# Arlo0o/StereoScene

Hardware: AMD Instinct MI355X
Metric: voxels/sec fwd+bwd, 256x256x32 grid D=192 (higher is better)
Workload: dtype f32; 1 GPU; kitti_d192: stereo pair features 2x[B,640,48,160] -> 256x256x32 occupancy, D=192, fwd+bwd incl. 4 losses; batch_per_gpu=1, global_batch=1, parallelism=dp1, train_mode=True

## Files before the change

include/ssbev.h:

```cpp
#ifndef SSBEV_H
#define SSBEV_H

#include <stddef.h>
#include <stdint.h>

#ifdef __cplusplus
extern "C" {
#endif

#define SSBEV_OK 0
#define SSBEV_EINVAL (-1)
#define SSBEV_EWORKSPACE (-2)
#define SSBEV_ELAUNCH (-3)

typedef void* ssbev_stream_t;

int ssbev_version(void);
const char* ssbev_build_arch(void);
void ssbev_env_refresh(void);

typedef struct {
  int B;
  int P;
  int C;
// ... 337 lines not shown
size_t ssbev_wino_dgemm_packed_elems(int Cout, int Cin);
int ssbev_wino_dgemm_pack(const float* w, float* Wp, int Cout, int Cin, int mode, ssbev_stream_t stream);
int ssbev_wino_dgemm(const float* P, const float* Wp, float* Mo, const ssbev_wino_dims* d, int N, ssbev_stream_t stream);
int ssbev_wino_bgemm(const float* A, const float* Wp, float* Cm, int64_t T, int K, int N, ssbev_stream_t stream);

typedef struct {
  int M, N, K, batch;
  int64_t lda, ldb, ldc, sa, sb, sc;
  int relu;
  int d2s_D, d2s_H, d2s_W, d2s_kd, d2s_kh, d2s_kw, d2s_Co;
  const int64_t* d2s_rowoff;
  const float* ep_mul;
  const float* ep_rowsub;
} ssbev_gemm_dims;
int ssbev_gemm_d2s_rowoff(int64_t* rowoff, int M, int D, int H, int W, int kd, int kh, int kw, int Co, ssbev_stream_t stream);
size_t ssbev_gemm_nn_workspace(const ssbev_gemm_dims* d);
size_t ssbev_gemm_nt_workspace(const ssbev_gemm_dims* d);
int ssbev_gemm_nn(const float* A, const float* B, const float* bias, float* C, const ssbev_gemm_dims* d, void* workspace,
                  size_t ws_bytes, ssbev_stream_t stream);
int ssbev_gemm_nt(const float* A, const float* W, const float* bias, float* C, const ssbev_gemm_dims* d, void* workspace,
                  size_t ws_bytes, ssbev_stream_t stream);
size_t ssbev_gemm_tn_workspace(const ssbev_gemm_dims* d);
int ssbev_gemm_tn(const float* A, const float* B, float* C, const ssbev_gemm_dims* d, void* workspace, size_t ws_bytes,
                  ssbev_stream_t stream);
typedef struct {
  int kernel;
  int bm, bn, bk;
  int nchunk;
  int per_chunk;
  int64_t grid;
  size_t workspace;
} ssbev_gemm_plan;
int ssbev_gemm_plan_query(const ssbev_gemm_dims* d, int form, ssbev_gemm_plan* out);

int ssbev_wino43_df_supported(const ssbev_wino_dims* d, int N);
int ssbev_wino43_df_instance(const ssbev_wino_dims* d, int N);
size_t ssbev_wino43_df_packed_elems(int Cout, int Cin);
int ssbev_wino43_df_pack(const float* w, float* Wp, int Cout, int Cin, int mode, ssbev_stream_t stream);
int ssbev_wino43_df_gemm(const float* P, const float* Wp, float* Mo, const ssbev_wino_dims* d, int N, ssbev_stream_t stream);
size_t ssbev_wino43_df_wgrad_workspace(const ssbev_wino_dims* d, int N);
int ssbev_wino43_df_wgrad(const float* P, const float* Z, float* gw, const ssbev_wino_dims* d, int N, void* workspace,
                          size_t ws_bytes, ssbev_stream_t stream);
typedef struct {
  int mt, nw;
  int ncolgrp, nrowgrp;
  int nst;
  int64_t grid;
  size_t lds_bytes;
  int w_kw, w_nt, w_br;
  int w_nkb, w_nnb;
  int w_nchunk;
  int w_stages_per_chunk;
  int w_total_stages;
  int64_t w_grid;
  size_t w_lds_bytes;
  size_t w_workspace;
} ssbev_wino43_df_plan;
int ssbev_wino43_df_plan_query(const ssbev_wino_dims* d, int N, ssbev_wino43_df_plan* out);

#ifdef __cplusplus
}
#endif
#endif
```

stereoscene_amd/capi.py:

```python
import ctypes as C
import os

import torch

_HERE = os.path.dirname(os.path.abspath(__file__))
LIB_PATH = os.path.join(_HERE, "_lib", "libssbev_hip.so")

OK, EINVAL, EWORKSPACE, ELAUNCH = 0, -1, -2, -3
_ERR = {EINVAL: "SSBEV_EINVAL (bad dims / null pointer / unsupported configuration)",
        EWORKSPACE: "SSBEV_EWORKSPACE (workspace too small)",
        ELAUNCH: "SSBEV_ELAUNCH (HIP launch failure)"}


class SsbevError(RuntimeError):
    pass


class PoolDims(C.Structure):
    _fields_ = [("B", C.c_int), ("P", C.c_int), ("C", C.c_int), ("nx", C.c_int), ("ny", C.c_int), ("nz", C.c_int),
                ("origin", C.c_float * 3), ("dx", C.c_float * 3)]


class LiftDims(C.Structure):
    _fields_ = [("N", C.c_int), ("D", C.c_int), ("HW", C.c_int)]
# ... 178 lines not shown
    "ssbev_depth_bce_fwd": (C.c_int, [_P, _P, _P] + [C.c_int] * 5 + [C.c_float] * 3 + [_P, C.c_size_t, _P]),
    "ssbev_depth_bce_bwd": (C.c_int, [_P, _P, _P, _P] + [C.c_int] * 5 + [C.c_float] * 3 + [_P, _P]),
    "ssbev_depth_kld_workspace": (C.c_size_t, [C.c_int, C.c_int, C.c_int]),
    "ssbev_depth_kld_fwd": (C.c_int, [_P, _P, _P] + [C.c_int] * 5 + [C.c_double] * 3 + [C.c_float] * 3 + [_P, C.c_size_t, _P]),
    "ssbev_depth_kld_bwd": (C.c_int, [_P, _P, _P, _P] + [C.c_int] * 5 + [C.c_double] * 3 + [C.c_float] * 3 + [_P, C.c_size_t, _P]),
    "ssbev_lidar_depth_workspace": (C.c_size_t, [C.c_int, C.c_int]),
    "ssbev_lidar_depth_map": (C.c_int, [_P, C.c_int, _P, _P, _P, _P, _P, _P, C.c_int, C.c_int, _P, C.c_size_t, _P]),
    "ssbev_dwconv2d_fwd": (C.c_int, [_P, _P, _P, C.POINTER(DwDims), _P]),
    "ssbev_dwconv2d_bwd_data": (C.c_int, [_P, _P, _P, C.POINTER(DwDims), _P]),
    "ssbev_dwconv2d_bwd_weight_workspace": (C.c_size_t, [C.POINTER(DwDims)]),
    "ssbev_dwconv2d_bwd_weight": (C.c_int, [_P, _P, _P, C.POINTER(DwDims), _P, C.c_size_t, _P]),
    "ssbev_swish_fwd": (C.c_int, [_P, _P, C.c_int64, _P]),
    "ssbev_swish_bwd": (C.c_int, [_P, _P, _P, C.c_int64, _P]),
    "ssbev_chan_sum_workspace": (C.c_size_t, [C.c_int, C.c_int64, C.c_int]),
    "ssbev_chan_sum": (C.c_int, [_P, _P, _P, C.c_int, C.c_int64, C.c_int, C.c_float, _P, C.c_size_t, _P]),
    "ssbev_chan_scale": (C.c_int, [_P, _P, _P, C.c_int, C.c_int64, C.c_int, C.c_float, _P]),
    "ssbev_wino_input_transform": (C.c_int, [_P, _P, C.POINTER(WinoDims), _P]),
    "ssbev_wino_output_transform": (C.c_int, [_P, _P, C.POINTER(WinoDims), _P]),
    "ssbev_wino_output_adjoint": (C.c_int, [_P, _P, C.POINTER(WinoDims), _P]),
    "ssbev_wino_weight_transform": (C.c_int, [_P, _P, C.c_int, C.c_int, C.c_int, C.c_int, _P]),
    "ssbev_wino_weight_grad": (C.c_int, [_P, _P, C.c_int, C.c_int, C.c_int, _P]),
    "ssbev_wino_dgemm_packed_elems": (C.c_size_t, [C.c_int, C.c_int]),
    "ssbev_wino_dgemm_pack": (C.c_int, [_P, _P, C.c_int, C.c_int, C.c_int, _P]),
    "ssbev_wino_dgemm": (C.c_int, [_P, _P, _P, C.POINTER(WinoDims), C.c_int, _P]),
    "ssbev_wino_bgemm": (C.c_int, [_P, _P, _P, C.c_int64, C.c_int, C.c_int, _P]),
    "ssbev_gemm_d2s_rowoff": (C.c_int, [_P, C.c_int, C.c_int, C.c_int, C.c_int, C.c_int, C.c_int, C.c_int, C.c_int, _P]),
    "ssbev_gemm_nn_workspace": (C.c_size_t, [C.POINTER(GemmDims)]),
    "ssbev_gemm_nt_workspace": (C.c_size_t, [C.POINTER(GemmDims)]),
    "ssbev_gemm_nn": (C.c_int, [_P, _P, _P, _P, C.POINTER(GemmDims), _P, C.c_size_t, _P]),
    "ssbev_gemm_nt": (C.c_int, [_P, _P, _P, _P, C.POINTER(GemmDims), _P, C.c_size_t, _P]),
    "ssbev_gemm_tn_workspace": (C.c_size_t, [C.POINTER(GemmDims)]),
    "ssbev_gemm_tn": (C.c_int, [_P, _P, _P, C.POINTER(GemmDims), _P, C.c_size_t, _P]),
    "ssbev_gemm_plan_query": (C.c_int, [C.POINTER(GemmDims), C.c_int, C.POINTER(GemmPlan)]),
    "ssbev_wino43_df_supported": (C.c_int, [C.POINTER(WinoDims), C.c_int]),
    "ssbev_wino43_df_instance": (C.c_int, [C.POINTER(WinoDims), C.c_int]),
    "ssbev_wino43_df_packed_elems": (C.c_size_t, [C.c_int, C.c_int]),
    "ssbev_wino43_df_pack": (C.c_int, [_P, _P, C.c_int, C.c_int, C.c_int, _P]),
    "ssbev_wino43_df_gemm": (C.c_int, [_P, _P, _P, C.POINTER(WinoDims), C.c_int, _P]),
    "ssbev_wino43_df_wgrad_workspace": (C.c_size_t, [C.POINTER(WinoDims), C.c_int]),
    "ssbev_wino43_df_wgrad": (C.c_int, [_P, _P, _P, C.POINTER(WinoDims), C.c_int, _P, C.c_size_t, _P]),
    "ssbev_wino43_df_plan_query": (C.c_int, [C.POINTER(WinoDims), C.c_int, C.POINTER(Wino43DfPlan)]),
    "ssbev_wino2d_axis_tiles": (C.c_int, [C.c_int, C.c_int, C.POINTER(C.c_uint16), C.c_int]),
    "ssbev_wino2d_input_transform": (C.c_int, [_P, _P, C.POINTER(WinoDims), _P]),
    "ssbev_wino2d_output_transform": (C.c_int, [_P, _P, C.POINTER(WinoDims), _P]),
    "ssbev_wino2d_output_adjoint": (C.c_int, [_P, _P, C.POINTER(WinoDims), _P]),
    "ssbev_wino43_input_transform": (C.c_int, [_P, _P, C.POINTER(WinoDims), _P]),
    "ssbev_wino43_input_transform_bf16": (C.c_int, [_P, _P, C.POINTER(WinoDims), _P]),
    "ssbev_wino43_output_transform": (C.c_int, [_P, _P, C.POINTER(WinoDims), _P]),
    "ssbev_wino43_output_transform_bf16": (C.c_int, [_P, _P, C.POINTER(WinoDims), _P]),
    "ssbev_wino43_output_adjoint": (C.c_int, [_P, _P, C.POINTER(WinoDims), _P]),
    "ssbev_wino43_output_adjoint_bf16": (C.c_int, [_P, _P, C.POINTER(WinoDims), _P]),
    "ssbev_wino43_2d_input_transform": (C.c_int, [_P, _P, C.POINTER(WinoDims), _P]),
    "ssbev_wino43_2d_input_transform_bf16": (C.c_int, [_P, _P, C.POINTER(WinoDims), _P]),
    "ssbev_wino43_2d_output_transform": (C.c_int, [_P, _P, C.POINTER(WinoDims), _P]),
    "ssbev_wino43_2d_output_transform_acc": (C.c_int, [_P, _P, C.POINTER(WinoDims), _P]),
    "ssbev_wino2d_output_transform_acc": (C.c_int, [_P, _P, C.POINTER(WinoDims), _P]),
    "ssbev_wino43_2d_output_transform_bf16": (C.c_int, [_P, _P, C.POINTER(WinoDims), _P]),
    "ssbev_wino43_2d_output_adjoint": (C.c_int, [_P, _P, C.POINTER(WinoDims), _P]),
    "ssbev_wino43_2d_output_adjoint_bf16": (C.c_int, [_P, _P, C.POINTER(WinoDims), _P]),
    "ssbev_wino444_input_transform": (C.c_int, [_P, _P, C.POINTER(WinoDims), _P]),
    "ssbev_wino444_output_transform": (C.c_int, [_P, _P, C.POINTER(WinoDims), _P]),
    "ssbev_wino444_output_adjoint": (C.c_int, [_P, _P, C.POINTER(WinoDims), _P]),
    "ssbev_wino43_weight_transform": (C.c_int, [_P, _P, C.c_int, C.c_int, C.c_int, C.c_int, _P]),
    "ssbev_wino43_weight_grad": (C.c_int, [_P, _P, C.c_int, C.c_int, C.c_int, _P]),
    "ssbev_wino_input_transform_bf16": (C.c_int, [_P, _P, C.POINTER(WinoDims), _P]),
    "ssbev_wino_output_transform_bf16": (C.c_int, [_P, _P, C.POINTER(WinoDims), _P]),
# ... 86 lines not shown
```

stereoscene_amd/csrc/capi.hip:

```cpp
#include "common.h"

#include <cstdlib>
#include <mutex>
#include <string>
#include <unordered_map>

namespace {
struct EnvTable {
  std::mutex mu;
  std::unordered_map<std::string, std::pair<bool, std::string>> seen;
};
EnvTable& env_table() {
  static EnvTable* t = new EnvTable();
  return *t;
}
}

const char* ssbev_env(const char* name) {
  EnvTable& t = env_table();
  std::lock_guard<std::mutex> lock(t.mu);
  auto it = t.seen.find(name);
  if (it == t.seen.end()) {
    const char* v = std::getenv(name);
    it = t.seen.emplace(name, std::make_pair(v != nullptr, std::string(v ? v : ""))).first;
  }
  return it->second.first ? it->second.second.c_str() : nullptr;
}

extern "C" {
int ssbev_version(void) { return 112;  }
const char* ssbev_build_arch(void) { return "gfx950"; }

void ssbev_env_refresh(void) {
  EnvTable& t = env_table();
  std::lock_guard<std::mutex> lock(t.mu);
  t.seen.clear();
}
}
```

stereoscene_amd/csrc/gemm.hip:

```cpp
#include "common.h"

#include <algorithm>
#include <cstdlib>
#include <string>

namespace {

typedef float gf32x16 __attribute__((ext_vector_type(16)));
typedef float gv4f __attribute__((ext_vector_type(4)));
__device__ const float kGemmZeros[4] = {0.f, 0.f, 0.f, 0.f};

struct GemmGeom {
  int M, N, K, batch;
  long lda, ldb, ldc;
  long sa, sb, sc;
  int mblocks, nblocks;
  int nchunk, rows_per_chunk;
  int relu;
  int d2s_D, d2s_H, d2s_W, d2s_kd, d2s_kh, d2s_kw, d2s_Co;
  const long* rowoff;
  const float* ep_mul;
  const float* ep_rowsub;
};

// ... 364 lines not shown
      for (int kt = 0; kt < KT; ++kt)
#pragma unroll
        for (int r = 0; r < 16; ++r) {
          const int k = ko + kt * 32 + (r & 3) + 8 * (r >> 2) + 4 * lk;
          if (k < g.K && n < g.N) dst[(size_t)k * g.N + n] = acc[kt][nt][r];
        }
    }
    return;
  }
  __shared__ float fold[QUAD ? 1 : 4][KT * NT * 1024];
#pragma unroll
  for (int kt = 0; kt < KT; ++kt)
#pragma unroll
    for (int nt = 0; nt < NT; ++nt)
#pragma unroll
      for (int r = 0; r < 16; ++r) fold[wave][((kt * NT + nt) * 16 + r) * 64 + lane] = acc[kt][nt][r];
  __syncthreads();
  if (wave != 0) return;
#pragma unroll
  for (int nt = 0; nt < NT; ++nt) {
    const int n = nt * 32 + li;
#pragma unroll
    for (int kt = 0; kt < KT; ++kt)
#pragma unroll
      for (int r = 0; r < 16; ++r) {
        const int k = kt * 32 + (r & 3) + 8 * (r >> 2) + 4 * lk;
        const int o = ((kt * NT + nt) * 16 + r) * 64 + lane;
        const float v = ((fold[0][o] + fold[1][o]) + fold[2][o]) + fold[3][o];
        if (k < g.K && n < g.N) dst[(size_t)k * g.N + n] = v;
      }
  }
}

__global__ void __launch_bounds__(1024)
gemm_sum_wide_kernel(const float* __restrict__ part, float* __restrict__ out, size_t n, int nchunk) {
  __shared__ float red[16][64];
  const int e = threadIdx.x & 63, grp = threadIdx.x >> 6;
  const size_t i = (size_t)blockIdx.x * 64 + e;
  const int per = (nchunk + 15) / 16, c0 = grp * per, c1 = min(nchunk, c0 + per);
  float a = 0.0f;
  if (i < n)
    for (int c = c0; c < c1; ++c) a += part[(size_t)c * n + i];
  red[grp][e] = a;
  __syncthreads();
  if (grp == 0 && i < n) {
    float v = red[0][e];
#pragma unroll
    for (int q = 1; q < 16; ++q) v += red[q][e];
    out[i] = v;
  }
}

__global__ void __launch_bounds__(256)
gemm_sum_kernel(const float* __restrict__ part, float* __restrict__ out, size_t n, int nchunk, const float* __restrict__ bias,
                int N, int relu, long MN = 0, long ldc = 0, long sc = 0) {
  const size_t i = (size_t)blockIdx.x * 256 + threadIdx.x;
  if (i >= n) return;
  float a = part[i];
  for (int c = 1; c < nchunk; ++c) a += part[(size_t)c * n + i];
  if (bias) a += bias[i % N];
  if (relu) a = fmaxf(a, 0.0f);
  if (MN > 0) {
    const size_t b = i / MN, r = i - b * MN;
    out[b * sc + (r / N) * ldc + r % N] = a;
  } else {
    out[i] = a;
// ... 157 lines not shown

LaunchPlan plan_tn(const ssbev_gemm_dims* d) {
  LaunchPlan pl;
  if (tn_skinny(d)) {
    const int wgs = tn_skinny_wgs(d);
    const bool quad = tn_quad(d);
    const long runs = quad ? wgs : (long)wgs * 4;
    const int kt = quad ? 2 : (d->K + 31) / 32, nt = quad ? 2 : (d->N + 31) / 32;
    pl.mblocks = pl.nblocks = 1;
    pl.p.kernel = quad ? kTnSkinnyQuad : (kt == 1 ? (nt == 1 ? kTnSkinny11 : kTnSkinny12) : (nt == 1 ? kTnSkinny21 : kTnSkinny22));
    pl.p.bm = (quad ? 64 : 32) * kt; pl.p.bn = (quad ? 64 : 32) * nt; pl.p.bk = 16;
    pl.p.nchunk = wgs;
    pl.p.per_chunk = (int)(((long)d->M + runs - 1) / runs + 1) / 2 * 2;
    pl.p.grid = (int64_t)wgs * d->batch;
    pl.p.workspace = (size_t)wgs * d->batch * d->K * d->N * sizeof(float);
    return pl;
  }
  const int wn = pick_wn(d->N, d->d2s_kd > 0 ? d->d2s_Co : 0);
  const bool wide = tn_wide(d);
  const int BN = wide ? 160 : 64 * wn;
  pl.mblocks = (d->K + 127) / 128;
  pl.nblocks = (d->N + BN - 1) / BN;
  const int tiles = pl.mblocks * pl.nblocks;
  const int nchunk = d->ep_mul ? 1 : (wide ? tn_chunks_model(d, tiles) : tn_chunks(d, tiles));
  pl.p.kernel = wide ? kTnWide : (wn == 2 ? kTnPlain : kTnNarrow);
  pl.p.bm = 128; pl.p.bn = BN; pl.p.bk = 32;
  pl.p.nchunk = nchunk;
  pl.p.per_chunk = ((d->M + nchunk - 1) / nchunk + 31) / 32 * 32;
  pl.p.grid = (int64_t)d->batch * nchunk * tiles;
  pl.p.workspace = nchunk > 1 ? (size_t)nchunk * d->batch * d->K * d->N * sizeof(float) : 0;
  return pl;
}

bool nn_dims_ok(const ssbev_gemm_dims* d) {
  if (!gemm_ok(d) || d->lda < d->K || d->ldb < d->N) return false;
  return d->d2s_kd > 0 ? (d->batch == 1 && d->N == d->d2s_kd * d->d2s_kh * d->d2s_kw * d->d2s_Co) : d->ldc >= d->N;
}
bool nt_dims_ok(const ssbev_gemm_dims* d) {
  if (!gemm_ok(d) || d->ldb < d->K || d->ldc < d->N) return false;
  return d->d2s_kd > 0 ? (d->batch == 1 && d->K == d->d2s_kd * d->d2s_kh * d->d2s_kw * d->d2s_Co) : d->lda >= d->K;
}
bool tn_dims_ok(const ssbev_gemm_dims* d) {
  if (!gemm_ok(d) || d->lda < d->K) return false;
  if (d->d2s_kd > 0 ? (d->batch != 1 || d->N != d->d2s_kd * d->d2s_kh * d->d2s_kw * d->d2s_Co) : d->ldb < d->N) return false;
  if ((d->ep_mul != nullptr) != (d->ep_rowsub != nullptr)) return false;
  return !(d->ep_mul && (tn_skinny(d) || d->d2s_kd > 0));
}

template <bool BT>
int launch_nn(const float* A, const float* B, const float* bias, float* Cm, const ssbev_gemm_dims* d, void* ws, size_t ws_bytes,
              hipStream_t st) {
  GemmGeom g;
  fill_geom(g, d);
  const LaunchPlan pl = plan_nn<BT>(d);
  const int cfg = pl.p.kernel;
  const NnCfg& c = kNnCfgs[cfg];
  g.mblocks = pl.mblocks;
  g.nblocks = pl.nblocks;
  g.nchunk = pl.p.nchunk;
  g.rows_per_chunk = pl.p.per_chunk;
  float* dst = Cm;
  const float* kbias = bias;
  if (g.nchunk > 1) {
    if (!ws || ws_bytes < pl.p.workspace) return SSBEV_EWORKSPACE;
    dst = static_cast<float*>(ws);
    g.ldc = d->N; g.sc = (long)d->M * d->N; g.relu = 0;
// ... 83 lines not shown
      default: hipLaunchKernelGGL((gemm_tn_skinny_kernel<2, 2, false>), grid, block, 0, st, A, B, part, g, rows_per_run); break;
    }
    const size_t n = (size_t)d->batch * d->K * d->N;
    hipLaunchKernelGGL(gemm_sum_wide_kernel, dim3(cdiv(n, 64)), dim3(1024), 0, st, part, Cm, n, wgs);
    return ssbev_launch_status();
  }
  g.mblocks = pl.mblocks;
  g.nblocks = pl.nblocks;
  g.nchunk = pl.p.nchunk;
  g.rows_per_chunk = pl.p.per_chunk;
  float* dst = g.nchunk > 1 ? static_cast<float*>(ws) : Cm;
  const long nwg = (long)pl.p.grid;
  const size_t lds = (size_t)2 * (32 * 128 + 32 * pl.p.bn) * sizeof(float);
  if (pl.p.kernel == kTnWide) {
    auto kern = gemm_tn_kernel<5, 1, 1>;
    if (hipFuncSetAttribute(reinterpret_cast<const void*>(kern), hipFuncAttributeMaxDynamicSharedMemorySize, (int)lds) != hipSuccess)
      return SSBEV_ELAUNCH;
    hipLaunchKernelGGL(kern, dim3((unsigned)nwg), dim3(256), lds, st, A, B, dst, g);
  } else if (pl.p.kernel == kTnPlain) {
    auto kern = gemm_tn_kernel<2>;
    if (hipFuncSetAttribute(reinterpret_cast<const void*>(kern), hipFuncAttributeMaxDynamicSharedMemorySize, (int)lds) != hipSuccess)
      return SSBEV_ELAUNCH;
    hipLaunchKernelGGL(kern, dim3((unsigned)nwg), dim3(256), lds, st, A, B, dst, g);
  } else {
    hipLaunchKernelGGL(gemm_tn_kernel<1>, dim3((unsigned)nwg), dim3(256), lds, st, A, B, dst, g);
  }
  if (g.nchunk > 1) {
    const size_t n = (size_t)g.batch * d->K * d->N;
    hipLaunchKernelGGL(gemm_sum_kernel, dim3(cdiv(n, 256)), dim3(256), 0, st, dst, Cm, n, g.nchunk, (const float*)nullptr, 1, 0);
  }
  return ssbev_launch_status();
}

int ssbev_gemm_plan_query(const ssbev_gemm_dims* d, int form, ssbev_gemm_plan* out) {
  if (!out) return SSBEV_EINVAL;
  switch (form) {
    case 0: if (!nn_dims_ok(d)) return SSBEV_EINVAL; *out = plan_nn<false>(d).p; return SSBEV_OK;
    case 1: if (!nt_dims_ok(d)) return SSBEV_EINVAL; *out = plan_nn<true>(d).p; return SSBEV_OK;
    case 2: if (!tn_dims_ok(d)) return SSBEV_EINVAL; *out = plan_tn(d).p; return SSBEV_OK;
    default: return SSBEV_EINVAL;
  }
}

}
```

stereoscene_amd/functional.py:

```python
import ctypes as C
import math

import os

import numpy as np
import torch

from . import capi, streams



class KernelTimer:

    def __init__(self, families=None):
        self.records = []
        self.counts = {}
        self.families = families

    def span(self, family, flops, nbytes=0.0, tag=None, executed=None):
        c = self.counts.setdefault(family, dict(launches=0, flops=0.0, bytes=0.0, executed=0.0))
        c["launches"] += 1
        c["flops"] += flops
        c["bytes"] += nbytes
        c["executed"] += flops if executed is None else executed
# ... 508 lines not shown

    @staticmethod
    def backward(ctx, gy):
        lib = capi.load()
        xcl, weight = ctx.saved_tensors[:2]
        stride, padding, dilation, transposed, output_padding, kpad, has_bias = ctx.cfg
        args = (stride, padding, dilation, transposed, output_padding)
        if ctx.relu:
            ycl = ctx.saved_tensors[2]
            gy = from_cl(torch.ops.aten.threshold_backward(to_cl(gy).contiguous(), ycl, 0.0))
        gcl0 = to_cl(gy)
        Cout_g = gcl0.shape[-1]
        cpad = (-Cout_g) % 4
        tpad = (-xcl.shape[-1]) % 4 if ctx.thin_in else 0
        want_gx, want_gw = ctx.needs_input_grad[0], ctx.needs_input_grad[1]
        thin_d = thin_w = False
        d0 = None
        if not transposed and not kpad and (cpad or tpad):
            d0 = _conv_dims(tuple(xcl.shape), tuple(weight.shape), *args)
            thin_d = bool(cpad) and lib.ssbev_conv_kernel_class(C.byref(d0), 1) == 4
            thin_w = lib.ssbev_conv_kernel_class(C.byref(d0), 2) == 6
        w5 = weight.detach()
        if kpad:
            w5 = torch.nn.functional.pad(w5, (0, 0, 0, 0, 0, 0) + ((0, 0, 0, kpad) if transposed else (0, kpad)))
        gcl = gcl0
        if cpad and ((want_gx and not thin_d) or (want_gw and not thin_w)):
            gcl = torch.nn.functional.pad(gcl0, (0, cpad))
            w5 = torch.nn.functional.pad(w5, (0, 0, 0, 0, 0, 0) + ((0, cpad) if transposed else (0, 0, 0, cpad)))
        elif cpad:
            w5 = None
        d = _conv_dims(tuple(xcl.shape), tuple(w5.shape), *args) if w5 is not None else d0
        gx = gw = gb = None

        def weight_gradient():
            pointwise = (not transposed and tuple(weight.shape[2:]) == (1, 1, 1) and stride == (1, 1, 1) and padding == (0, 0, 0)
                         and not kpad and not cpad and not tpad and weight.shape[0] <= 128 and weight.shape[1] <= 128
                         and gcl0.numel() // Cout_g >= 32768)
            if pointwise and OWN_GEMM and PRECISION == "fp32":
                with _span("conv_wgrad", conv_flops(d), conv_bytes(d), _conv_tag(d, "wgrad")):
                    gw = gemm_tn(gcl0.reshape(-1, Cout_g), xcl.reshape(-1, xcl.shape[-1])).view_as(weight)
            else:
                if thin_w:
                    xw, gw_src, dw, wshape = xcl, gcl0, d0, tuple(weight.shape)
                else:
                    xw, gw_src, dw, wshape = xcl, gcl, d, tuple(w5.shape)
                    if tpad:
                        xw = torch.nn.functional.pad(xcl, (0, tpad))
                        wshape = (wshape[0], wshape[1] + tpad) + wshape[2:]
                        dw = _conv_dims(tuple(xw.shape), wshape, *args)
                gwp = torch.empty(wshape, dtype=torch.float32, device=gy.device)
                ws = _ws(lib.ssbev_conv_bwd_weight_workspace(C.byref(dw)), gy.device)
                with _span("conv_wgrad", conv_flops(dw), conv_bytes(dw), _conv_tag(dw, "wgrad")):
                    capi.check(lib.ssbev_conv_bwd_weight(capi.ptr(xw), capi.ptr(gw_src), capi.ptr(gwp), C.byref(dw),
                                                         capi.ptr(ws), ws.numel(), capi.stream()),
                               "ssbev_conv_bwd_weight")
                gw = gwp if tuple(wshape) == tuple(weight.shape) else gwp[: weight.shape[0], : weight.shape[1]].contiguous()
            return gw

        gw_side = want_gw and streams.wgrad_on_side(weight)
        want_gb = has_bias and ctx.needs_input_grad[2]
        gb_side = gw_side and want_gb and ctx.bias_leaf
        if gw_side:
            with streams.on_side(gy.device, xcl, gcl0, gcl) as side:
                gw = weight_gradient()
                if gb_side:
                    gb = gcl0.reshape(-1, Cout_g).sum(0)
                side.publish(gw, gb)
        if want_gx:
            dd, gdl, wd = (d0, gcl0, weight.detach()) if thin_d else (d, gcl, w5)
            slot = ctx.slot if (not kpad and not thin_d and lib.ssbev_conv_kernel_class(C.byref(dd), 1) not in (4, 5)) else None
            into = _slot_target(slot, xcl)
            if into is not None:
                dd.accumulate = 1
            gxcl = into if into is not None else torch.empty_like(xcl)
            fam = _conv_family(lib, dd, 1)
            with _span(fam, conv_flops(dd), conv_bytes(dd), _conv_tag(dd, "dgrad"), conv_flops(dd) / _EXEC_DIV[fam]):
                if lib.ssbev_conv_kernel_class(C.byref(dd), 1) == 5:
                    _thin_out_run(lib, gdl, wd, None, gxcl, dd, 1)
                else:
                    wpt = _packed(wd, dd, 1)
                    capi.check(lib.ssbev_conv_bwd_data(capi.ptr(gdl), capi.ptr(wpt), capi.ptr(gxcl), C.byref(dd),
                                                       capi.stream()), "ssbev_conv_bwd_data")
            dd.accumulate = 0
            if slot is not None:
                slot.buf = gxcl
            if kpad:
                gxcl = gxcl[..., : xcl.shape[-1] - kpad]
            gx = from_cl(gxcl)
        if want_gw and not gw_side:
            gw = weight_gradient()
        if want_gb and not gb_side:
            gb = gcl0.reshape(-1, Cout_g).sum(0)
        return gx, gw, gb, None, None, None, None, None, None, None


class _ConvNd16(torch.autograd.Function):

    @staticmethod
    def forward(ctx, x, weight, bias, stride, padding, dilation, transposed, output_padding, slot=None, relu=False, out_fp32=False):
        lib = capi.load()
        ctx.slot = slot
        if ctx.needs_input_grad[1]:
            streams.note_use(weight)
        xcl = to_cl(x if x.dtype == torch.bfloat16 else x.to(torch.bfloat16))
        d = _conv_dims(tuple(xcl.shape), tuple(weight.shape), stride, padding, dilation, transposed, output_padding, relu=int(relu))
        d.precision = 3 if out_fp32 else 2
        y = torch.empty(d.B, d.Do, d.Ho, d.Wo, d.Cout, dtype=torch.float32 if out_fp32 else torch.bfloat16, device=x.device)
        b = bias.detach().float().contiguous() if bias is not None else None
        fam = {17: "conv_tap16", 19: "conv_wide16"}.get(lib.ssbev_conv_kernel_class(C.byref(d), 0), "conv_gather16") if KERNEL_TIMER is not None else "conv_gather16"
        with _span(fam, conv_flops(d), conv_bytes(d) / 2.0, _conv_tag(d, "fwd")):
            wp = _packed(weight.detach(), d, 0)
            capi.check(lib.ssbev_conv_fwd_bf16(capi.ptr(xcl), capi.ptr(wp), capi.ptr(b), capi.ptr(y), C.byref(d), capi.stream()),
                       "ssbev_conv_fwd_bf16")
        ctx.relu = bool(relu)
        ctx.save_for_backward(xcl, weight, *((y,) if relu else ()))
        ctx.cfg = (stride, padding, dilation, transposed, output_padding, bias is not None)
        ctx.bias_leaf = bias is not None and bias.is_leaf and bias.grad is None
        return from_cl(y)

    @staticmethod
    def backward(ctx, gy):
        lib = capi.load()
        xcl, weight = ctx.saved_tensors[:2]
        stride, padding, dilation, transposed, output_padding, has_bias = ctx.cfg
# ... 199 lines not shown
    lib = capi.load()
    ws = _ws(lib.ssbev_gemm_nt_workspace(C.byref(g)), a.device)
    with _span("gemm_own", fl, 4.0 * (a.numel() + w.numel() + out.numel()), tag or f"nt {batch}x{M}x{K}x{N}"):
        capi.check(lib.ssbev_gemm_nt(_rawptr(a), _rawptr(w), _rawptr(bias.contiguous() if bias is not None else None),
                                     capi.ptr(out), C.byref(g), capi.ptr(ws), ws.numel(), capi.stream()), "ssbev_gemm_nt")
    return out


def gemm_tn(a, b, tag=None, ep_mul=None, ep_rowsub=None):
    if not _gemm_supported(a, b) or a.shape[-1] % 4 or b.shape[-1] % 4:
        c = torch.matmul(a.transpose(-1, -2), b)
        return c if ep_mul is None else ep_mul * (c - ep_rowsub.unsqueeze(-1))
    a, lda, sa = _rows(a)
    b, ldb, sb = _rows(b)
    batch = a.shape[0] if a.dim() == 3 else 1
    R, K, N = a.shape[-2], a.shape[-1], b.shape[-1]
    out = torch.empty(*a.shape[:-2], K, N, dtype=torch.float32, device=a.device)
    g = _gdims(R, N, K, batch, lda, ldb, N, sa, sb, K * N)
    if ep_mul is not None:
        ep_mul, ep_rowsub = ep_mul.contiguous(), ep_rowsub.contiguous().float()
        if tuple(ep_mul.shape) != tuple(out.shape) or ep_rowsub.numel() != batch * K:
            raise capi.SsbevError("gemm_tn: epilogue operand shapes")
        g.ep_mul, g.ep_rowsub = ep_mul.data_ptr(), ep_rowsub.data_ptr()
    lib = capi.load()
    ws = _ws(lib.ssbev_gemm_tn_workspace(C.byref(g)), a.device)
    fl = 2.0 * batch * R * N * K
    with _span("gemm_own", fl, 4.0 * (a.numel() + b.numel() + out.numel() * (2 if ep_mul is not None else 1)),
               tag or f"tn {batch}x{R}x{K}x{N}"):
        capi.check(lib.ssbev_gemm_tn(_rawptr(a), _rawptr(b), capi.ptr(out), C.byref(g), capi.ptr(ws), ws.numel(), capi.stream()),
                   "ssbev_gemm_tn")
    return out


class _LinearCL(torch.autograd.Function):

    @staticmethod
    def forward(ctx, x2, w2, bias):
        ctx.save_for_backward(x2, w2)
        ctx.has_bias = bias is not None
        return gemm_nt(x2, w2, bias, tag=f"linear fwd {w2.shape[1]}->{w2.shape[0]} rows={x2.shape[0]}")

    @staticmethod
    def backward(ctx, gy):
        x2, w2 = ctx.saved_tensors
        gy = gy.contiguous()
        gx = gw = gb = None
        if ctx.needs_input_grad[0]:
            gx = gemm_nn(gy, w2, tag=f"linear dgrad {w2.shape[1]}->{w2.shape[0]} rows={x2.shape[0]}")
        if ctx.needs_input_grad[1]:
            gw = gemm_tn(gy, x2, tag=f"linear wgrad {w2.shape[1]}->{w2.shape[0]} rows={x2.shape[0]}")
        if ctx.has_bias and ctx.needs_input_grad[2]:
            gb = gy.sum(0)
        return gx, gw, gb


_D2S_TABLES = {}


def _d2s_table(B, D, H, W, k, Co, device):
    key = (B, D, H, W, k, Co, str(device))
    t = _D2S_TABLES.get(key)
    if t is None:
        t = torch.empty(B * D * H * W, dtype=torch.int64, device=device)
        capi.check(capi.load().ssbev_gemm_d2s_rowoff(capi.ptr(t), B * D * H * W, D, H, W, k[0], k[1], k[2], Co, capi.stream()),
                   "ssbev_gemm_d2s_rowoff")
        _D2S_TABLES[key] = t
    return t


class _DeconvKS(torch.autograd.Function):

    @staticmethod
    def forward(ctx, xcl, weight, bias, k):
        B, D, H, W, Ci = xcl.shape
        Co = weight.shape[1]
        kd, kh, kw = k
        taps = kd * kh * kw
        wk = weight.detach().permute(0, 2, 3, 4, 1).reshape(Ci, taps * Co).contiguous()
        table = _d2s_table(B, D, H, W, k, Co, xcl.device)
        y = torch.empty(B, D * kd, H * kh, W * kw, Co, dtype=torch.float32, device=xcl.device)
        x2 = xcl.reshape(-1, Ci)
        R = x2.shape[0]
        g = _gdims(R, taps * Co, Ci, 1, Ci, taps * Co, 0, 0, 0, 0, 0, ((D, H, W, kd, kh, kw, Co), table))
        fl = 2.0 * R * Ci * taps * Co
# ... 1669 lines not shown
```

Baseline: 31.26 million voxels/s.

## Add fused pointwise weight-gradient kernel with bias-gradient column sums

Measured after the change: 31.28 million voxels/s, median of 6. No clear change (+0.1%).

```diff
diff --git a/include/ssbev.h b/include/ssbev.h
--- a/include/ssbev.h
+++ b/include/ssbev.h
@@ -393,6 +393,10 @@
   size_t workspace;
 } ssbev_gemm_plan;
 int ssbev_gemm_plan_query(const ssbev_gemm_dims* d, int form, ssbev_gemm_plan* out);
+size_t ssbev_wgrad_pointwise_workspace(const ssbev_gemm_dims* d);
+int ssbev_wgrad_pointwise_plan(const ssbev_gemm_dims* d, ssbev_gemm_plan* out);
+int ssbev_wgrad_pointwise(const float* A, const float* B, float* gw, float* gb, int gy_operand, const ssbev_gemm_dims* d,
+                          void* workspace, size_t ws_bytes, ssbev_stream_t stream);
 
 int ssbev_wino43_df_supported(const ssbev_wino_dims* d, int N);
 int ssbev_wino43_df_instance(const ssbev_wino_dims* d, int N);
diff --git a/stereoscene_amd/capi.py b/stereoscene_amd/capi.py
--- a/stereoscene_amd/capi.py
+++ b/stereoscene_amd/capi.py
@@ -234,6 +234,9 @@
     "ssbev_gemm_tn_workspace": (C.c_size_t, [C.POINTER(GemmDims)]),
     "ssbev_gemm_tn": (C.c_int, [_P, _P, _P, C.POINTER(GemmDims), _P, C.c_size_t, _P]),
     "ssbev_gemm_plan_query": (C.c_int, [C.POINTER(GemmDims), C.c_int, C.POINTER(GemmPlan)]),
+    "ssbev_wgrad_pointwise_workspace": (C.c_size_t, [C.POINTER(GemmDims)]),
+    "ssbev_wgrad_pointwise_plan": (C.c_int, [C.POINTER(GemmDims), C.POINTER(GemmPlan)]),
+    "ssbev_wgrad_pointwise": (C.c_int, [_P, _P, _P, _P, C.c_int, C.POINTER(GemmDims), _P, C.c_size_t, _P]),
     "ssbev_wino43_df_supported": (C.c_int, [C.POINTER(WinoDims), C.c_int]),
     "ssbev_wino43_df_instance": (C.c_int, [C.POINTER(WinoDims), C.c_int]),
     "ssbev_wino43_df_packed_elems": (C.c_size_t, [C.c_int, C.c_int]),
diff --git a/stereoscene_amd/csrc/capi.hip b/stereoscene_amd/csrc/capi.hip
--- a/stereoscene_amd/csrc/capi.hip
+++ b/stereoscene_amd/csrc/capi.hip
@@ -28,7 +28,7 @@
 }
 
 extern "C" {
-int ssbev_version(void) { return 112;  }
+int ssbev_version(void) { return 113;  }
 const char* ssbev_build_arch(void) { return "gfx950"; }
 
 void ssbev_env_refresh(void) {
diff --git a/stereoscene_amd/csrc/gemm.hip b/stereoscene_amd/csrc/gemm.hip
--- a/stereoscene_amd/csrc/gemm.hip
+++ b/stereoscene_amd/csrc/gemm.hip
@@ -420,6 +420,231 @@
   }
 }
 
+template <int KT, int NT, int WK, int WN>
+struct WgradPw {
+  static constexpr bool SHARED = WK * WN == 4;
+  static constexpr int KC = 32 * KT * WK, NC = 32 * NT * WN;
+  static constexpr int RS = SHARED ? ((KC == 32 || NC == 32) ? 32 : 16) : (KT * NT == 1 ? 16 : 8);
+  static constexpr int RW = SHARED ? RS / 4 : RS;
+  static constexpr int AF = RS * KC, BF = RS * NC, SF = AF + BF;
+  static constexpr int AP = RW * KC / 256, BP = RW * NC / 256, IPS = AP + BP;
+  static constexpr int NBUF = 3;
+  static constexpr int TILE = KT * NT * 1024;
+  static constexpr int STAGE_FLOATS = (SHARED ? 1 : 4) * NBUF * SF;
+  static constexpr int FOLD_FLOATS = SHARED ? 0 : 3 * TILE + 4 * (KC + NC);
+  static constexpr int LDS_FLOATS = STAGE_FLOATS > FOLD_FLOATS ? STAGE_FLOATS : FOLD_FLOATS;
+  static constexpr int UNIT = SHARED ? RS : 4 * RS;
+  static_assert(WK * WN == 1 || WK * WN == 4, "one wave or four per staging unit");
+  static_assert((RW * KC) % 256 == 0 && (RW * NC) % 256 == 0 && IPS <= 15, "a wave copies whole 1 KiB pieces");
+};
+
+template <int KT, int NT, int WK, int WN>
+__global__ void __launch_bounds__(256)
+wgrad_pw_kernel(const float* __restrict__ A, const float* __restrict__ B, float* __restrict__ part, GemmGeom g, int rows_per_wg,
+                int bias_sel) {
+  using P = WgradPw<KT, NT, WK, WN>;
+  constexpr bool SHARED = P::SHARED;
+  constexpr int KC = P::KC, NC = P::NC, RS = P::RS, RW = P::RW, AF = P::AF, SF = P::SF, AP = P::AP, BP = P::BP, IPS = P::IPS;
+  extern __shared__ __align__(16) float lds[];
+  const int tid = threadIdx.x, lane = tid & 63, wave = __builtin_amdgcn_readfirstlane(tid >> 6);
+  const int li = lane & 31, lk = lane >> 5;
+  const int wk = SHARED ? wave / WN : 0, wn = SHARED ? wave % WN : 0;
+  const int wg = xcd_logical(blockIdx.x, gridDim.x);
+  long r_begin = (long)wg * rows_per_wg, r_end = min((long)g.M, r_begin + rows_per_wg);
+  if (!SHARED) {
+    const int per = rows_per_wg >> 2;
+    r_begin += (long)wave * per;
+    r_end = min(r_end, r_begin + per);
+  }
+  int rem = r_end > r_begin ? (int)(r_end - r_begin) : 0;
+  const int nst = (rem + RS - 1) / RS;
+  float* mine = lds + (SHARED ? 0 : wave * (P::NBUF * SF));
+  const int rbase = SHARED ? wave * RW : 0;
+
+  const float* ap[AP]; int ar[AP]; bool ac[AP];
+#pragma unroll
+  for (int e = 0; e < AP; ++e) {
+    const int k = (lane % (KC / 4)) * 4;
+    ar[e] = e * (256 / KC) + lane / (KC / 4);
+    ac[e] = k < g.K;
+    ap[e] = A + (r_begin + rbase + ar[e]) * g.lda + k;
+  }
+  const float* bp[BP]; int br[BP]; bool bc[BP];
+#pragma unroll
+  for (int e = 0; e < BP; ++e) {
+    const int n = (lane % (NC / 4)) * 4;
+    br[e] = e * (256 / NC) + lane / (NC / 4);
+    bc[e] = n < g.N;
+    bp[e] = B + (r_begin + rbase + br[e]) * g.ldb + n;
+  }
+  const long astep = (long)RS * g.lda, bstep = (long)RS * g.ldb;
+  auto issue = [&](int buf) {
+    float* dst = mine + buf * SF + rbase * KC;
+#pragma unroll
+    for (int e = 0; e < AP; ++e) {
+      glds16((ac[e] && rbase + ar[e] < rem) ? ap[e] : kGemmZeros, dst + e * 256);
+      ap[e] += astep;
+    }
+    dst = mine + buf * SF + AF + rbase * NC;
+#pragma unroll
+    for (int e = 0; e < BP; ++e) {
+      glds16((bc[e] && rbase + br[e] < rem) ? bp[e] : kGemmZeros, dst + e * 256);
+      bp[e] += bstep;
+    }
+    rem -= RS;
+  };
+
+  gf32x16 acc[KT][NT];
+#pragma unroll
+  for (int kt = 0; kt < KT; ++kt)
+#pragma unroll
+    for (int nt = 0; nt < NT; ++nt)
+#pragma unroll
+      for (int r = 0; r < 16; ++r) acc[kt][nt][r] = 0.0f;
+  float sa[KT], sb[NT];
+#pragma unroll
+  for (int kt = 0; kt < KT; ++kt) sa[kt] = 0.0f;
+#pragma unroll
+  for (int nt = 0; nt < NT; ++nt) sb[nt] = 0.0f;
+
+  if (nst > 0) issue(0);
+  if (nst > 1) issue(1);
+  int buf = 0;
+  for (int st = 0; st < nst; ++st) {
+    if (st + 1 < nst) asm volatile("s_waitcnt vmcnt(%0)" ::"n"(IPS) : "memory");
+    else asm volatile("s_waitcnt vmcnt(0)" ::: "memory");
+    if (SHARED) __builtin_amdgcn_s_barrier();
+    if (st + 2 < nst) issue(buf >= 1 ? buf - 1 : 2);
+    const float* as = mine + buf * SF + (wk * KT) * 32 + li;
+    const float* bs = mine + buf * SF + AF + (wn * NT) * 32 + li;
+    float av[KT], bv[NT], an[KT], bn[NT];
+    auto fetch = [&](int rp, float (&a)[KT], float (&b)[NT]) {
+      const int row = 2 * rp + lk;
+#pragma unroll
+      for (int kt = 0; kt < KT; ++kt) a[kt] = as[row * KC + kt * 32];
+#pragma unroll
+      for (int nt = 0; nt < NT; ++nt) b[nt] = bs[row * NC + nt * 32];
+    };
+    fetch(0, av, bv);
+#pragma unroll
+    for (int rp = 0; rp < RS / 2; ++rp) {
+      if (rp + 1 < RS / 2) fetch(rp + 1, an, bn);
+      __builtin_amdgcn_sched_barrier(0);
+#pragma unroll
+      for (int kt = 0; kt < KT; ++kt) sa[kt] += av[kt];
+#pragma unroll
+      for (int nt = 0; nt < NT; ++nt) sb[nt] += bv[nt];
+#pragma unroll
+      for (int kt = 0; kt < KT; ++kt)
+#pragma unroll
+        for (int nt = 0; nt < NT; ++nt)
+          acc[kt][nt] = __builtin_amdgcn_mfma_f32_32x32x2f32(av[kt], bv[nt], acc[kt][nt], 0, 0, 0);
+#pragma unroll
+      for (int kt = 0; kt < KT; ++kt) av[kt] = an[kt];
+#pragma unroll
+      for (int nt = 0; nt < NT; ++nt) bv[nt] = bn[nt];
+    }
+    asm volatile("s_waitcnt lgkmcnt(0)" ::: "memory");
+    buf = buf == 2 ? 0 : buf + 1;
+  }
+#pragma unroll
+  for (int kt = 0; kt < KT; ++kt) sa[kt] += __shfl_xor(sa[kt], 32);
+#pragma unroll
+  for (int nt = 0; nt < NT; ++nt) sb[nt] += __shfl_xor(sb[nt], 32);
+
+  const int nbias = bias_sel == 1 ? g.K : (bias_sel == 2 ? g.N : 0);
+  const size_t kn = (size_t)g.K * g.N;
+  float* dst = part + (size_t)wg * (kn + nbias);
+  if (SHARED) {
+#pragma unroll
+    for (int nt = 0; nt < NT; ++nt) {
+      const int n = (wn * NT + nt) * 32 + li;
+#pragma unroll
+      for (int kt = 0; kt < KT; ++kt)
+#pragma unroll
+        for (int r = 0; r < 16; ++r) {
+          const int k = (wk * KT + kt) * 32 + (r & 3) + 8 * (r >> 2) + 4 * lk;
+          if (k < g.K && n < g.N) dst[(size_t)k * g.N + n] = acc[kt][nt][r];
+        }
+    }
+    if (bias_sel == 1 && wn == 0 && lk == 0) {
+#pragma unroll
+      for (int kt = 0; kt < KT; ++kt) {
+        const int k = (wk * KT + kt) * 32 + li;
+        if (k < g.K) dst[kn + k] = sa[kt];
+      }
+    }
+    if (bias_sel == 2 && wk == 0 && lk == 0) {
+#pragma unroll
+      for (int nt = 0; nt < NT; ++nt) {
+        const int n = (wn * NT + nt) * 32 + li;
+        if (n < g.N) dst[kn + n] = sb[nt];
+      }
+    }
+    return;
+  }
+  constexpr int TILE = P::TILE;
+  float* fold = lds;
+  float* cs = lds + 3 * TILE;
+  __syncthreads();
+  if (wave != 0) {
+#pragma unroll
+    for (int kt = 0; kt < KT; ++kt)
+#pragma unroll
+      for (int nt = 0; nt < NT; ++nt)
+#pragma unroll
+        for (int r = 0; r < 16; ++r) fold[(wave - 1) * TILE + ((kt * NT + nt) * 16 + r) * 64 + lane] = acc[kt][nt][r];
+  }
+  if (lk == 0) {
+#pragma unroll
+    for (int kt = 0; kt < KT; ++kt) cs[wave * (KC + NC) + kt * 32 + li] = sa[kt];
+#pragma unroll
+    for (int nt = 0; nt < NT; ++nt) cs[wave * (KC + NC) + KC + nt * 32 + li] = sb[nt];
+  }
+  __syncthreads();
+  if (wave != 0) return;
+#pragma unroll
+  for (int nt = 0; nt < NT; ++nt) {
+    const int n = nt * 32 + li;
+#pragma unroll
+    for (int kt = 0; kt < KT; ++kt)
+#pragma unroll
+      for (int r = 0; r < 16; ++r) {
+        const int k = kt * 32 + (r & 3) + 8 * (r >> 2) + 4 * lk;
+        const int o = ((kt * NT + nt) * 16 + r) * 64 + lane;
+        const float v = ((acc[kt][nt][r] + fold[o]) + fold[TILE + o]) + fold[2 * TILE + o];
+        if (k < g.K && n < g.N) dst[(size_t)k * g.N + n] = v;
+      }
+  }
+  if (bias_sel != 0) {
+    const int off = bias_sel == 1 ? 0 : KC;
+    for (int c = lane; c < nbias; c += 64) {
+      const float* p = cs + off + c;
+      dst[kn + c] = ((p[0] + p[KC + NC]) + p[2 * (KC + NC)]) + p[3 * (KC + NC)];
+    }
+  }
+}
+
+__global__ void __launch_bounds__(1024)
+gemm_sum_wide2_kernel(const float* __restrict__ part, float* __restrict__ out, float* __restrict__ out2, size_t n, size_t n1,
+                      int nchunk) {
+  __shared__ float red[16][64];
+  const int e = threadIdx.x & 63, grp = threadIdx.x >> 6;
+  const size_t i = (size_t)blockIdx.x * 64 + e;
+  const int per = (nchunk + 15) / 16, c0 = grp * per, c1 = min(nchunk, c0 + per);
+  float a = 0.0f;
+  if (i < n)
+    for (int c = c0; c < c1; ++c) a += part[(size_t)c * n + i];
+  red[grp][e] = a;
+  __syncthreads();
+  if (grp == 0 && i < n) {
+    float v = red[0][e];
+#pragma unroll
+    for (int q = 1; q < 16; ++q) v += red[q][e];
+    if (i < n1) out[i] = v; else out2[i - n1] = v;
+  }
+}
+
 __global__ void __launch_bounds__(1024)
 gemm_sum_wide_kernel(const float* __restrict__ part, float* __restrict__ out, size_t n, int nchunk) {
   __shared__ float red[16][64];
@@ -643,6 +868,58 @@
   return pl;
 }
 
+enum { kWgradPw11 = 30, kWgradPw12 = 31, kWgradPw21 = 32, kWgradPw22 = 33, kWgradPwQuad = 34, kWgradPwTall1 = 35, kWgradPwTall2 = 36,
+       kWgradPwWide1 = 37, kWgradPwWide2 = 38 };
+
+bool wgrad_pw_dims_ok(const ssbev_gemm_dims* d) {
+  return gemm_ok(d) && d->batch == 1 && d->K <= 128 && d->N <= 128 && d->lda >= d->K && d->ldb >= d->N && d->d2s_kd == 0 &&
+         !d->ep_mul && !d->ep_rowsub;
+}
+
+template <int KT, int NT, int WK, int WN>
+void wgrad_pw_fill(ssbev_gemm_plan& p, int code) {
+  using P = WgradPw<KT, NT, WK, WN>;
+  p.kernel = code; p.bm = P::KC; p.bn = P::NC; p.bk = P::RS;
+  p.per_chunk = P::UNIT;
+}
+
+LaunchPlan plan_wgrad_pw(const ssbev_gemm_dims* d) {
+  LaunchPlan pl;
+  const int kc = (d->K + 31) / 32, nc = (d->N + 31) / 32;
+  if (kc <= 2 && nc <= 2) {
+    if (kc == 1) { if (nc == 1) wgrad_pw_fill<1, 1, 1, 1>(pl.p, kWgradPw11); else wgrad_pw_fill<1, 2, 1, 1>(pl.p, kWgradPw12); }
+    else { if (nc == 1) wgrad_pw_fill<2, 1, 1, 1>(pl.p, kWgradPw21); else wgrad_pw_fill<2, 2, 1, 1>(pl.p, kWgradPw22); }
+  } else if (kc > 2 && nc > 2) {
+    wgrad_pw_fill<2, 2, 2, 2>(pl.p, kWgradPwQuad);
+  } else if (kc > 2) {
+    if (nc == 1) wgrad_pw_fill<1, 1, 4, 1>(pl.p, kWgradPwTall1); else wgrad_pw_fill<1, 2, 4, 1>(pl.p, kWgradPwTall2);
+  } else {
+    if (kc == 1) wgrad_pw_fill<1, 1, 1, 4>(pl.p, kWgradPwWide1); else wgrad_pw_fill<2, 1, 1, 4>(pl.p, kWgradPwWide2);
+  }
+  const bool split = pl.p.kernel <= kWgradPw22;
+  const long unit = pl.p.per_chunk, target = split ? 768 : 512;
+  long per = ((long)d->M + target - 1) / target;
+  per = std::max(2 * unit, (per + unit - 1) / unit * unit);
+  const long wgs = ((long)d->M + per - 1) / per;
+  pl.mblocks = pl.nblocks = 1;
+  pl.p.per_chunk = (int)per;
+  pl.p.nchunk = (int)wgs;
+  pl.p.grid = wgs;
+  pl.p.workspace = (size_t)wgs * ((size_t)d->K * d->N + std::max(d->K, d->N)) * sizeof(float);
+  return pl;
+}
+
+template <int KT, int NT, int WK, int WN>
+int launch_wgrad_pw(const float* A, const float* B, float* part, const GemmGeom& g, const LaunchPlan& pl, int bias_sel, hipStream_t st) {
+  using P = WgradPw<KT, NT, WK, WN>;
+  auto kern = wgrad_pw_kernel<KT, NT, WK, WN>;
+  const size_t lds = (size_t)P::LDS_FLOATS * sizeof(float);
+  if (hipFuncSetAttribute(reinterpret_cast<const void*>(kern), hipFuncAttributeMaxDynamicSharedMemorySize, (int)lds) != hipSuccess)
+    return SSBEV_ELAUNCH;
+  hipLaunchKernelGGL(kern, dim3((unsigned)pl.p.grid), dim3(256), lds, st, A, B, part, g, pl.p.per_chunk, bias_sel);
+  return SSBEV_OK;
+}
+
 bool nn_dims_ok(const ssbev_gemm_dims* d) {
   if (!gemm_ok(d) || d->lda < d->K || d->ldb < d->N) return false;
   return d->d2s_kd > 0 ? (d->batch == 1 && d->N == d->d2s_kd * d->d2s_kh * d->d2s_kw * d->d2s_Co) : d->ldc >= d->N;
@@ -792,6 +1069,45 @@
   return ssbev_launch_status();
 }
 
+size_t ssbev_wgrad_pointwise_workspace(const ssbev_gemm_dims* d) { return wgrad_pw_dims_ok(d) ? plan_wgrad_pw(d).p.workspace : 0; }
+
+int ssbev_wgrad_pointwise_plan(const ssbev_gemm_dims* d, ssbev_gemm_plan* out) {
+  if (!out || !wgrad_pw_dims_ok(d)) return SSBEV_EINVAL;
+  *out = plan_wgrad_pw(d).p;
+  return SSBEV_OK;
+}
+
+int ssbev_wgrad_pointwise(const float* A, const float* B, float* gw, float* gb, int gy_operand, const ssbev_gemm_dims* d, void* ws,
+                          size_t ws_bytes, ssbev_stream_t stream) {
+  if (!wgrad_pw_dims_ok(d) || !A || !B || !gw || (gy_operand != 0 && gy_operand != 1)) return SSBEV_EINVAL;
+  if (((uintptr_t)A | (uintptr_t)B) & 15) return SSBEV_EINVAL;
+  const LaunchPlan pl = plan_wgrad_pw(d);
+  if (!ws || ws_bytes < pl.p.workspace) return SSBEV_EWORKSPACE;
+  GemmGeom g;
+  fill_geom(g, d);
+  g.ldc = d->N; g.sc = (long)d->K * d->N; g.relu = 0;
+  hipStream_t st = as_stream(stream);
+  float* part = static_cast<float*>(ws);
+  const int bias_sel = gb ? 1 + gy_operand : 0;
+  int rc;
+  switch (pl.p.kernel) {
+    case kWgradPw11: rc = launch_wgrad_pw<1, 1, 1, 1>(A, B, part, g, pl, bias_sel, st); break;
+    case kWgradPw12: rc = launch_wgrad_pw<1, 2, 1, 1>(A, B, part, g, pl, bias_sel, st); break;
+    case kWgradPw21: rc = launch_wgrad_pw<2, 1, 1, 1>(A, B, part, g, pl, bias_sel, st); break;
+    case kWgradPw22: rc = launch_wgrad_pw<2, 2, 1, 1>(A, B, part, g, pl, bias_sel, st); break;
+    case kWgradPwQuad: rc = launch_wgrad_pw<2, 2, 2, 2>(A, B, part, g, pl, bias_sel, st); break;
+    case kWgradPwTall1: rc = launch_wgrad_pw<1, 1, 4, 1>(A, B, part, g, pl, bias_sel, st); break;
+    case kWgradPwTall2: rc = launch_wgrad_pw<1, 2, 4, 1>(A, B, part, g, pl, bias_sel, st); break;
+    case kWgradPwWide1: rc = launch_wgrad_pw<1, 1, 1, 4>(A, B, part, g, pl, bias_sel, st); break;
+    case kWgradPwWide2: rc = launch_wgrad_pw<2, 1, 1, 4>(A, B, part, g, pl, bias_sel, st); break;
+    default: return SSBEV_EINVAL;
+  }
+  if (rc != SSBEV_OK) return rc;
+  const size_t kn = (size_t)d->K * d->N, n = kn + (bias_sel == 0 ? 0 : (bias_sel == 1 ? d->K : d->N));
+  hipLaunchKernelGGL(gemm_sum_wide2_kernel, dim3(cdiv(n, 64)), dim3(1024), 0, st, part, gw, gb, n, kn, pl.p.nchunk);
+  return ssbev_launch_status();
+}
+
 int ssbev_gemm_plan_query(const ssbev_gemm_dims* d, int form, ssbev_gemm_plan* out) {
   if (!out) return SSBEV_EINVAL;
   switch (form) {
diff --git a/stereoscene_amd/functional.py b/stereoscene_amd/functional.py
--- a/stereoscene_amd/functional.py
+++ b/stereoscene_amd/functional.py
@@ -564,13 +564,21 @@
         d = _conv_dims(tuple(xcl.shape), tuple(w5.shape), *args) if w5 is not None else d0
         gx = gw = gb = None
 
-        def weight_gradient():
+        def weight_gradient(with_gb=False):
+            nonlocal gb
             pointwise = (not transposed and tuple(weight.shape[2:]) == (1, 1, 1) and stride == (1, 1, 1) and padding == (0, 0, 0)
                          and not kpad and not cpad and not tpad and weight.shape[0] <= 128 and weight.shape[1] <= 128
                          and gcl0.numel() // Cout_g >= 32768)
             if pointwise and OWN_GEMM and PRECISION == "fp32":
                 with _span("conv_wgrad", conv_flops(d), conv_bytes(d), _conv_tag(d, "wgrad")):
-                    gw = gemm_tn(gcl0.reshape(-1, Cout_g), xcl.reshape(-1, xcl.shape[-1])).view_as(weight)
+                    gy2, x2 = gcl0.reshape(-1, Cout_g), xcl.reshape(-1, xcl.shape[-1])
+                    if wgrad_pointwise_applicable(gy2, x2, with_gb):
+                        gw, gb_pw = wgrad_pointwise(gy2, x2, 0 if with_gb else None)
+                        if with_gb:
+                            gb = gb_pw
+                    else:
+                        gw = gemm_tn(gy2, x2)
+                    gw = gw.view_as(weight)
             else:
                 if thin_w:
                     xw, gw_src, dw, wshape = xcl, gcl0, d0, tuple(weight.shape)
@@ -594,8 +602,8 @@
         gb_side = gw_side and want_gb and ctx.bias_leaf
         if gw_side:
             with streams.on_side(gy.device, xcl, gcl0, gcl) as side:
-                gw = weight_gradient()
-                if gb_side:
+                gw = weight_gradient(gb_side)
+                if gb_side and gb is None:
                     gb = gcl0.reshape(-1, Cout_g).sum(0)
                 side.publish(gw, gb)
         if want_gx:
@@ -620,8 +628,8 @@
                 gxcl = gxcl[..., : xcl.shape[-1] - kpad]
             gx = from_cl(gxcl)
         if want_gw and not gw_side:
-            gw = weight_gradient()
-        if want_gb and not gb_side:
+            gw = weight_gradient(want_gb and not gb_side)
+        if want_gb and gb is None:
             gb = gcl0.reshape(-1, Cout_g).sum(0)
         return gx, gw, gb, None, None, None, None, None, None, None
 
@@ -887,6 +895,32 @@
     return out
 
 
+WGRAD_PW_MIN_ROWS = 32768
+
+
+def wgrad_pointwise_applicable(a, b, want_gb=True):
+    if not (_gemm_supported(a, b) and PRECISION == "fp32" and a.dim() == 2 and b.dim() == 2 and a.shape[0] == b.shape[0]
+            and a.shape[0] >= WGRAD_PW_MIN_ROWS and a.shape[1] <= 128 and b.shape[1] <= 128
+            and a.shape[1] % 4 == 0 and b.shape[1] % 4 == 0):
+        return False
+    return want_gb or not (32 < max(a.shape[1], b.shape[1]) <= 64)
+
+
+def wgrad_pointwise(a, b, gy_operand=None, tag=None):
+    a, lda, _ = _rows(a)
+    b, ldb, _ = _rows(b)
+    R, K, N = a.shape[0], a.shape[1], b.shape[1]
+    gw = torch.empty(K, N, dtype=torch.float32, device=a.device)
+    gb = None if gy_operand is None else torch.empty(N if gy_operand else K, dtype=torch.float32, device=a.device)
+    g = _gdims(R, N, K, 1, lda, ldb, N, 0, 0, K * N)
+    lib = capi.load()
+    ws = _ws(lib.ssbev_wgrad_pointwise_workspace(C.byref(g)), a.device)
+    with _span("gemm_own", 2.0 * R * N * K, 4.0 * (a.numel() + b.numel() + gw.numel()), tag or f"tn 1x{R}x{K}x{N}"):
+        capi.check(lib.ssbev_wgrad_pointwise(_rawptr(a), _rawptr(b), capi.ptr(gw), capi.ptr(gb), int(gy_operand or 0), C.byref(g),
+                                             capi.ptr(ws), ws.numel(), capi.stream()), "ssbev_wgrad_pointwise")
+    return gw, gb
+
+
 class _LinearCL(torch.autograd.Function):
 
     @staticmethod
@@ -902,9 +936,14 @@
         gx = gw = gb = None
         if ctx.needs_input_grad[0]:
             gx = gemm_nn(gy, w2, tag=f"linear dgrad {w2.shape[1]}->{w2.shape[0]} rows={x2.shape[0]}")
+        want_gb = ctx.has_bias and ctx.needs_input_grad[2]
         if ctx.needs_input_grad[1]:
-            gw = gemm_tn(gy, x2, tag=f"linear wgrad {w2.shape[1]}->{w2.shape[0]} rows={x2.shape[0]}")
-        if ctx.has_bias and ctx.needs_input_grad[2]:
+            tag = f"linear wgrad {w2.shape[1]}->{w2.shape[0]} rows={x2.shape[0]}"
+            if wgrad_pointwise_applicable(gy, x2, want_gb):
+                gw, gb = wgrad_pointwise(gy, x2, 0 if want_gb else None, tag=tag)
+            else:
+                gw = gemm_tn(gy, x2, tag=tag)
+        if want_gb and gb is None:
             gb = gy.sum(0)
         return gx, gw, gb
 
```
